# MisterPup/PDE-MultiGrid

Measured on AMD Instinct MI355X. Metric: MLUPS on 3D Poisson 512^3 V-cycle, higher is better.
Workload: dtype f64

## Files before the change

### include/mgx.h

```cpp
#ifndef MGX_H
#define MGX_H

#include <stddef.h>
#include <stdint.h>

#ifdef __cplusplus
extern "C" {
#endif

typedef enum {
    MGX_OK = 0,
    MGX_ERR_INVALID = 1,
    MGX_ERR_SIZE = 2,
    MGX_ERR_HIP = 3,
    MGX_ERR_NOMEM = 4,
    MGX_ERR_RCCL = 5,
    MGX_ERR_NOGPU = 6
} mgx_status;

typedef enum { MGX_RESIDUAL_REF_COMPAT = 0, MGX_RESIDUAL_CORRECT = 1 } mgx_residual_mode;

typedef struct mgx_ctx mgx_ctx;
typedef struct mgx_event mgx_event;

const char* mgx_status_string(int status);
const char* mgx_last_error(void);
void mgx_set_last_error(const char* msg);
const char* mgx_version(void);

int mgx_device_count(int* count);
int mgx_ctx_create(int device, mgx_ctx** out);
int mgx_ctx_destroy(mgx_ctx* ctx);
int mgx_ctx_sync(mgx_ctx* ctx);
int mgx_ctx_check(mgx_ctx* ctx);
int mgx_ctx_clear_abort(mgx_ctx* ctx, int reenable);
int mgx_ctx_generation(const mgx_ctx* ctx, unsigned long long* generation);
int mgx_ctx_prepare(mgx_ctx* ctx);
int mgx_ctx_device(const mgx_ctx* ctx, int* device);
int mgx_ctx_set_param(mgx_ctx* ctx, const char* name, int value);
const char* mgx_ctx_last_relax_kernel(const mgx_ctx* ctx);
const char* mgx_ctx_last_rr_kernel(const mgx_ctx* ctx);
const char* mgx_ctx_last_corr_kernel(const mgx_ctx* ctx);
int mgx_test_set_lds_poison(int on);
int mgx_test_lds_probe(mgx_ctx* ctx, double* fraction);
int mgx_ctx_stream(const mgx_ctx* ctx, void** hip_stream);

int mgx_malloc(mgx_ctx* ctx, size_t bytes, void** dptr);
int mgx_free(mgx_ctx* ctx, void* dptr);
int mgx_memcpy_h2d(mgx_ctx* ctx, void* dst, const void* host_src, size_t bytes);
int mgx_memcpy_d2h(mgx_ctx* ctx, void* host_dst, const void* src, size_t bytes);
int mgx_memcpy_d2d(mgx_ctx* ctx, void* dst, const void* src, size_t bytes);
int mgx_memset_zero(mgx_ctx* ctx, void* dst, size_t bytes);

int mgx_graph_begin(mgx_ctx* ctx);
int mgx_graph_end(mgx_ctx* ctx, void** graph_exec);
int mgx_graph_launch(mgx_ctx* ctx, void* graph_exec);
int mgx_graph_destroy(mgx_ctx* ctx, void* graph_exec);
int mgx_event_create(mgx_ctx* ctx, mgx_event** out);
int mgx_event_destroy(mgx_ctx* ctx, mgx_event* ev);
int mgx_event_record(mgx_ctx* ctx, mgx_event* ev);
int mgx_event_elapsed_ms(mgx_ctx* ctx, mgx_event* start, mgx_event* stop, float* ms);

#define MGX_DECLARE_OPS(SFX, real)                                                                      \
    int mgx3d_relax_##SFX(mgx_ctx* ctx, real* v, const real* f, const int n[3], const real h[3],        \
                          int ncycles);                                                                 \
     \
     \
     \
    int mgx3d_relax_from_zero_##SFX(mgx_ctx* ctx, real* v, const real* f, const int n[3], const real h[3], \
                                    int ncycles, int rim_is_zero);                                      \
    int mgx3d_residual_##SFX(mgx_ctx* ctx, const real* v, const real* f, real* r, const int n[3],       \
                             const real h[3], int mode);                                                \
    int mgx3d_restrict_##SFX(mgx_ctx* ctx, const real* fine, const int fn[3], real* coarse,             \
                             const int cn[3]);                                                          \
    int mgx3d_interpolate_##SFX(mgx_ctx* ctx, real* fine, const int fn[3], const real* coarse,          \
                                const int cn[3]);                                                       \
    int mgx3d_apply_correction_##SFX(mgx_ctx* ctx, real* fine, const int fn[3], const real* err,        \
                                     const int en[3]);                                                  \
    int mgx3d_set_##SFX(mgx_ctx* ctx, real* grid, const int n[3], real value, int modify_boundaries);   \
    int mgx3d_residual_restrict_##SFX(mgx_ctx* ctx, const real* v, const real* f, const int n[3],       \
                                      const real h[3], int mode, real* coarse_f, const int cn[3]);      \
     \
     \
    int mgx3d_residual_restrict_keep_rim_##SFX(mgx_ctx* ctx, const real* v, const real* f,              \
                                               const int n[3], const real h[3], int mode,               \
                                               real* coarse_f, const int cn[3]);                        \
    int mgx3d_interpolate_correct_##SFX(mgx_ctx* ctx, real* v, const int n[3], const real* coarse_v,    \
                                        const int cn[3]);                                               \
    int mgx3d_init_f_##SFX(mgx_ctx* ctx, real* f, const int n[3], double c, const double* host_tx,      \
                           const double* host_ty, const double* host_tz);                               \
    int mgx3d_jacobi_##SFX(mgx_ctx* ctx, real* v, real* tmp, const real* f, const int n[3],             \
                           const real h[3], real omega, int ncycles);                                   \
     \
     \
     \
// ... 286 lines not shown
```

### pde_multigrid_amd/_lib.py

```python
import ctypes as C
import os

_HERE = os.path.dirname(os.path.abspath(__file__))
LIB_PATH = os.environ.get("MGX_LIB_PATH") or os.path.join(_HERE, "lib", "libmgx.so")

MGX_OK, MGX_ERR_INVALID, MGX_ERR_SIZE, MGX_ERR_HIP, MGX_ERR_NOMEM, MGX_ERR_RCCL, MGX_ERR_NOGPU = range(7)
REF_COMPAT, CORRECT = 0, 1
UNIQUE_ID_BYTES = 128


class MgxError(RuntimeError):
    def __init__(self, status, message):
        super().__init__("%s: %s" % (status_string(status), message))
        self.status = status


if not os.path.exists(LIB_PATH):
    raise ImportError(
        "pde_multigrid_amd: %s is missing -- build it with `python -c 'import __graft_entry__ as g; g.build()'` "
        "or `make -C pde_multigrid_amd/csrc`; there is no CPU fallback for the HIP path" % LIB_PATH)

lib = C.CDLL(LIB_PATH, mode=C.RTLD_GLOBAL)
lib.mgx_status_string.restype = C.c_char_p
lib.mgx_last_error.restype = C.c_char_p
lib.mgx_version.restype = C.c_char_p
lib.mgx_ctx_last_relax_kernel.restype = C.c_char_p
lib.mgx_ctx_last_rr_kernel.restype = C.c_char_p
lib.mgx_ctx_last_corr_kernel.restype = C.c_char_p


def status_string(status):
    return lib.mgx_status_string(int(status)).decode()


def check(status):
    if status != MGX_OK:
        raise MgxError(status, lib.mgx_last_error().decode())
    return status
```

### pde_multigrid_amd/csrc/mgx_internal.hpp

```cpp
#pragma once
#include <hip/hip_runtime.h>

#include <cstdarg>
#include <cstdio>
#include <cstring>

#include "mgx.h"

struct mgx_ctx {
    int device = 0;
    hipStream_t compute = nullptr;
    hipStream_t comm = nullptr;
    hipEvent_t ev_compute = nullptr;
    hipEvent_t ev_comm = nullptr;
    int comm_inline = 0;
    int relax_ty = 4;
    int relax_zchunk = 0;
    int relax_xcd = 1;
    int rr_rows = 0;
    int rr_rcp = 1;
    int rr_xcd = 1;
    int relax_rows = 4;
    int relax_wave_planes = 0;
    int relax_small = 1;
    int relax_ablate = 0;
    int rr_stream = 3;
    int relax_lds = -1;
    int rr_cr = 0, rr_tyw = 4;
    int rr_pzchunk = 0;
    int rr_black = 1;
    int rr_black_abl = 0;
    int rr_black_waves = 0;
    int relax_zero_first = 1;
    int relax_zero_sweep = 1;
    int corr_v2 = 1;
    int relax_v2 = 1;
    int corr_fuse = 1;
    int cyc2_tile = 0;
    int cyc2_tail_points = 33 * 33;
    int sweep_fused = 0;
    int sweep_mid = 1;
    int relax_resident = 1;
    int relax_resident_min = 3;
    void* resident_buf = nullptr;
    size_t resident_bytes = 0;
    int sweep_ilv = 0;
    int sweep_lead = 0;
    int sweep_dbg = 0;
    void* sweep_dev = nullptr;
    unsigned* sweep_abort = nullptr;
    unsigned sync_spin_limit = 1u << 21;
    unsigned handoff_fault = 0;
    int handoff_broken = 0;
    unsigned long long generation = 0;
    int gpu_exclusive = 1;
    mutable int resident_occ = -1;
    void* scratch = nullptr;
    size_t scratch_bytes = 0;
    void* rccl_comm = nullptr;
    void* local_group = nullptr;
    int rank = 0, nranks = 1;
    int comm_rehearse = 0;
    void* rehearse_buf = nullptr;
    size_t rehearse_bytes = 0;
    int num_cus = 256;
    int pipe_unroll = 7;
    int corr_low = 0;
    int slab_edges_merged = 1;
    int resident_tile = 0;
    char last_corr_kernel[96] = "";
    char last_rr_kernel[96] = "";
    char last_relax_kernel[96] = "";
};

struct mgx_event {
    hipEvent_t ev = nullptr;
};

namespace mgx {

void set_error(const char* fmt, ...);

inline int fail(int status, const char* fmt, ...) {
    char buf[512];
    va_list ap;
    va_start(ap, fmt);
    vsnprintf(buf, sizeof buf, fmt, ap);
    va_end(ap);
    set_error("%s", buf);
    return status;
}

int workspace(mgx_ctx* ctx, size_t bytes, void** out);
int fill_zero(mgx_ctx* ctx, void* dst, size_t bytes);

inline int ceil_div(long long a, long long b) { return (int)((a + b - 1) / b); }

template <class real>
inline void note_relax_kernel(mgx_ctx* ctx, const char* name, int a, int b, int c, bool fnt = false) {
    snprintf(ctx->last_relax_kernel, sizeof ctx->last_relax_kernel, "%s<%s,%d,%d,%d%s>", name, sizeof(real) == 8 ? "double" : "float",
             a, b, c, fnt ? ",true" : "");
}

inline bool valid_size(int n) { return n >= 3 && ((n - 1) % 2 == 0); }

struct SmallDiv {
    int d;
    float r;
    __host__ __device__ explicit SmallDiv(int d_) : d(d_), r(1.0f / (float)d_) {}
    __device__ __forceinline__ int operator()(int t) const {
        int q = (int)((float)t * r);
        const int rem = t - q * d;
        q += (rem >= d) - (rem < 0);
        return q;
    }
};

}

#define MGX_HIP(expr)                                                                         \
    do {                                                                                      \
        hipError_t e_ = (expr);                                                               \
        if (e_ != hipSuccess)                                                                 \
            return mgx::fail(MGX_ERR_HIP, "%s failed: %s (%s:%d)", #expr, hipGetErrorString(e_), \
                             __FILE__, __LINE__);                                             \
// ... 24 lines not shown
```

### pde_multigrid_amd/csrc/mgx_kernels3d.hip

```cpp
#include <type_traits>

#include "mgx_internal.hpp"
#include "mgx_kernels3d.hpp"
#include "mgx_sync.hpp"

namespace mgx {

template <class real>
__global__ void __launch_bounds__(256) relax3d_colour_kernel(real* __restrict__ v, const real* __restrict__ f, int sx,
                                                             int sy, int sz, real hx2, real hy2, real hz2, int colour) {
    const int y = 1 + blockIdx.y * blockDim.y + threadIdx.y;
    const int z = 1 + blockIdx.z;
    if (y >= sy - 1) return;
    const int p = (colour + y + z) & 1;
    const int x = 2 * (blockIdx.x * blockDim.x + threadIdx.x) + p;
    if (x < 1 || x >= sx - 1) return;
    const size_t sxy = (size_t)sx * sy;
    const size_t i = x + (size_t)y * sx + (size_t)z * sxy;
    const real O = v[i - 1], E = v[i + 1];
    const real N = v[i - sx], S = v[i + sx];
    const real D = v[i - sxy], U = v[i + sxy];
    v[i] = relax3d_point<real>(O, E, N, S, D, U, f[i], hx2, hy2, hz2);
}

// ... 2514 lines not shown
        else if (TYWr == 2) MGX_RR(M, C, 2);       \
        else MGX_RR(M, C, 4);                      \
    } while (0)
    if (mode == MGX_RESIDUAL_REF_COMPAT) {
        if (rcp) { if (CRr == 1) MGX_RR_W(2, 1); else MGX_RR_W(2, 2); }
        else { if (CRr == 1) MGX_RR_W(0, 1); else MGX_RR_W(0, 2); }
    } else {
        if (rcp) { if (CRr == 1) MGX_RR_W(3, 1); else MGX_RR_W(3, 2); }
        else { if (CRr == 1) MGX_RR_W(1, 1); else MGX_RR_W(1, 2); }
    }
#undef MGX_RR_W
#undef MGX_RR
    return MGX_OK;
}

template <class real, class L>
int residual_restrict3d(mgx_ctx* ctx, const real* v, const real* f, const int n[3], const real h[3], int mode,
                        real* coarse_f, const int cn[3], bool rim_is_zero = false) {
    MGX_REQUIRE(ctx && v && f && h && coarse_f, MGX_ERR_INVALID, "residual_restrict3d: NULL argument");
    MGX_USE(ctx);
    int st = check_n3(n, "residual_restrict3d");
    if (st) return st;
    st = check_coarse3(n, cn, "residual_restrict3d");
    if (st) return st;
    MGX_REQUIRE(mode == MGX_RESIDUAL_REF_COMPAT || mode == MGX_RESIDUAL_CORRECT, MGX_ERR_INVALID,
                "residual_restrict3d: bad mode %d", mode);
    const real hx2 = h[0] * h[0], hy2 = h[1] * h[1], hz2 = h[2] * h[2];
    if (L::xsplit && ctx->rr_stream) {
        st = residual_restrict3d_xs_launch<real>(ctx, v, f, n, hx2, hy2, hz2, mode, coarse_f, cn, 0, 0, 0, cn[2], rim_is_zero);
        if (st) return st;
        MGX_LAUNCH_CHECK();
        return MGX_OK;
    }
    constexpr int CTX = 32, CTY = 8;
    const int tiles = ceil_div(cn[0], CTX) * ceil_div(cn[1], CTY);
    int pzchunk = ctx->rr_pzchunk > 0 ? ctx->rr_pzchunk : 8;
    while (pzchunk > 1 && (long long)tiles * ceil_div(cn[2], pzchunk) < 4LL * ctx->num_cus) pzchunk >>= 1;
    dim3 g(ceil_div(cn[0], CTX), ceil_div(cn[1], CTY), ceil_div(cn[2], pzchunk));
    if (mode == MGX_RESIDUAL_REF_COMPAT)
        MGX_LAUNCH((residual_restrict3d_kernel<real, L, 0, CTX, CTY>), g, blk(), 0, ctx->compute, v, f, n[0], n[1],
                           n[2], hx2, hy2, hz2, coarse_f, cn[0], cn[1], cn[2], pzchunk, 0, 0, 0, cn[2]);
    else
        MGX_LAUNCH((residual_restrict3d_kernel<real, L, 1, CTX, CTY>), g, blk(), 0, ctx->compute, v, f, n[0], n[1],
                           n[2], hx2, hy2, hz2, coarse_f, cn[0], cn[1], cn[2], pzchunk, 0, 0, 0, cn[2]);
    MGX_LAUNCH_CHECK();
    return MGX_OK;
}

bool relax_rr3d_xs_takes(const mgx_ctx* ctx, const int n[3], const int cn[3], size_t elem);
template <class real>
bool relax_rr3d_xs_launch(mgx_ctx* ctx, real* v, const real* f, const int n[3], real hx2, real hy2, real hz2, int mode, bool rcp,
                          real* coarse_f, const int cn[3], int fzoff, int czoff, int pzbeg, int pzend);

template <class real>
int relax_rr3d_slab(mgx_ctx* ctx, real* v, const real* f, const int n[3], int fzoff, const real h[3], int mode, real* coarse_f,
                    const int cn[3], int czoff, int pzbeg, int pzend) {
    MGX_REQUIRE(ctx && v && f && h && coarse_f, MGX_ERR_INVALID, "relax_rr_slab: NULL argument");
    MGX_USE(ctx);
    int st = check_n3(n, "relax_rr_slab");
    if (st) return st;
    st = check_coarse3(n, cn, "relax_rr_slab");
    if (st) return st;
    MGX_REQUIRE(mode == MGX_RESIDUAL_REF_COMPAT || mode == MGX_RESIDUAL_CORRECT, MGX_ERR_INVALID, "relax_rr_slab: bad mode %d", mode);
    MGX_REQUIRE(pzbeg >= 1 && pzend <= cn[2] - 1 && pzbeg < pzend && czoff >= 0 && czoff <= pzbeg && fzoff >= 0 && (fzoff & 1) == 0 &&
                    fzoff <= (2 * pzbeg - 3 > 0 ? 2 * pzbeg - 3 : 0),
                MGX_ERR_INVALID, "relax_rr_slab: coarse planes [%d, %d) with offsets %d / %d", pzbeg, pzend, fzoff, czoff);
    MGX_REQUIRE(relax_rr3d_xs_takes(ctx, n, cn, sizeof(real)), MGX_ERR_INVALID, "relax_rr_slab: the level is not taken (ask relax_rr_takes)");
    const real hx2 = h[0] * h[0], hy2 = h[1] * h[1], hz2 = h[2] * h[2];
    const Geo<XSplit, real> gc(cn[0], cn[1]);
    MGX_TRY_RET(fill_zero(ctx, coarse_f + gc.PL * (size_t)(pzbeg - czoff), gc.PL * (size_t)(pzend - pzbeg) * sizeof(real)));
    const bool rcp = ctx->rr_rcp && exact_reciprocal(hx2) && exact_reciprocal(hy2) && exact_reciprocal(hz2);
    MGX_REQUIRE(relax_rr3d_xs_launch<real>(ctx, v, f, n, hx2, hy2, hz2, mode, rcp, coarse_f, cn, fzoff, czoff, pzbeg, pzend), MGX_ERR_INVALID,
                "relax_rr_slab: launch refused");
    MGX_LAUNCH_CHECK();
    return MGX_OK;
}

template <class real>
int smooth_residual_restrict3d_xs(mgx_ctx* ctx, real* v, const real* f, const int n[3], const real h[3], int ncycles, int from_zero,
                                  int v_rim_is_zero, int mode, real* coarse_f, const int cn[3], int coarse_rim_is_zero) {
    MGX_REQUIRE(ctx && v && f && h && coarse_f, MGX_ERR_INVALID, "smooth_residual_restrict3d: NULL argument");
    MGX_USE(ctx);
    int st = check_n3(n, "smooth_residual_restrict3d");
    if (st) return st;
    st = check_coarse3(n, cn, "smooth_residual_restrict3d");
    if (st) return st;
    MGX_REQUIRE(ncycles >= 0, MGX_ERR_INVALID, "smooth_residual_restrict3d: ncycles = %d < 0", ncycles);
    MGX_REQUIRE(mode == MGX_RESIDUAL_REF_COMPAT || mode == MGX_RESIDUAL_CORRECT, MGX_ERR_INVALID,
                "smooth_residual_restrict3d: bad mode %d", mode);
    ctx->last_rr_kernel[0] = 0;
    if (ncycles < 1 || !relax_rr3d_xs_takes(ctx, n, cn, sizeof(real))) {
        st = from_zero ? relax3d_from_zero<real, XSplit>(ctx, v, f, n, h, ncycles, v_rim_is_zero) : relax3d<real, XSplit>(ctx, v, f, n, h, ncycles);
        if (st) return st;
        return residual_restrict3d<real, XSplit>(ctx, v, f, n, h, mode, coarse_f, cn, coarse_rim_is_zero != 0);
    }
    const real hx2 = h[0] * h[0], hy2 = h[1] * h[1], hz2 = h[2] * h[2];
    int s = 0;
    if (from_zero) {
        if (v_rim_is_zero && ctx->relax_zero_first) {
            if (2 * ncycles - 1 >= 2 && relax3d_xs_first_sweep_zero<real>(ctx, v, f, n[0], n[1], n[2], hx2, hy2, hz2)) {
                s = 2;
            } else {
                MGX_LAUNCH((relax3d_zero_colour_kernel<real, XSplit>), dim3(ceil_div((n[0] + 1) / 2, 64), ceil_div(n[1] - 2, 4), n[2] - 2),
                                   blk(), 0, ctx->compute, v, f, n[0], n[1], hx2, hy2, hz2, 0, 1);
                s = 1;
            }
        } else {
            MGX_TRY_RET(fill_zero(ctx, v, Geo<XSplit, real>(n[0], n[1]).PL * (size_t)n[2] * sizeof(real)));
        }
    }
    for (; s < 2 * ncycles - 1; s++) relax3d_xs_pass<real>(ctx, v, f, n[0], n[1], 1, n[2] - 1, hx2, hy2, hz2, s & 1);
    if (!coarse_rim_is_zero) MGX_TRY_RET(fill_zero(ctx, coarse_f, Geo<XSplit, real>(cn[0], cn[1]).PL * (size_t)cn[2] * sizeof(real)));
    const bool rcp = ctx->rr_rcp && exact_reciprocal(hx2) && exact_reciprocal(hy2) && exact_reciprocal(hz2);
    MGX_REQUIRE(relax_rr3d_xs_launch<real>(ctx, v, f, n, hx2, hy2, hz2, mode, rcp, coarse_f, cn, 0, 0, 1, cn[2] - 1), MGX_ERR_INVALID,
                "smooth_residual_restrict3d: the fused launch refused a level it had accepted");
    MGX_LAUNCH_CHECK();
    return MGX_OK;
}

template <class real, class L>
int init_f3d(mgx_ctx* ctx, real* f, const int n[3], double c, const double* tx, const double* ty, const double* tz) {
    MGX_REQUIRE(ctx && f && tx && ty && tz, MGX_ERR_INVALID, "init_f3d: NULL argument");
    MGX_USE(ctx);
    int st = check_n3(n, "init_f3d");
    if (st) return st;
    const size_t cnt = (size_t)n[0] + n[1] + n[2];
    void* ws = nullptr;
    st = workspace(ctx, cnt * sizeof(double), &ws);
    if (st) return st;
    double* d = (double*)ws;
    MGX_HIP(hipMemcpyAsync(d, tx, n[0] * sizeof(double), hipMemcpyHostToDevice, ctx->compute));
    MGX_HIP(hipMemcpyAsync(d + n[0], ty, n[1] * sizeof(double), hipMemcpyHostToDevice, ctx->compute));
    MGX_HIP(hipMemcpyAsync(d + n[0] + n[1], tz, n[2] * sizeof(double), hipMemcpyHostToDevice, ctx->compute));
    MGX_LAUNCH((init_f3d_kernel<real, L>), grd(n[0], n[1], n[2]), blk(), 0, ctx->compute, f, n[0], n[1], n[2], c, d,
                       d + n[0], d + n[0] + n[1]);
    MGX_LAUNCH_CHECK();
    MGX_HIP(hipStreamSynchronize(ctx->compute));
    return MGX_OK;
}

template <class real, class LS, class LD>
int relayout3d(mgx_ctx* ctx, const real* src, real* dst, const int n[3]) {
    MGX_REQUIRE(ctx && src && dst, MGX_ERR_INVALID, "relayout3d: NULL argument");
    MGX_USE(ctx);
    MGX_REQUIRE(src != dst, MGX_ERR_INVALID, "relayout3d: in-place conversion is not supported");
    int st = check_n3(n, "relayout3d");
    if (st) return st;
    MGX_LAUNCH((relayout3d_kernel<real, LS, LD>), grd(n[0], n[1], n[2]), blk(), 0, ctx->compute, src, dst, n[0], n[1]);
    MGX_LAUNCH_CHECK();
    return MGX_OK;
}

template <class real>
int relax3d_colour_slab(mgx_ctx* ctx, real* v, const real* f, int sx, int sy, const real h[3], int colour, int zbeg,
                        int zend, int zoff) {
    MGX_REQUIRE(ctx && v && f && h, MGX_ERR_INVALID, "relax_colour_slab: NULL argument");
    MGX_USE(ctx);
    MGX_REQUIRE(valid_size(sx) && valid_size(sy), MGX_ERR_SIZE, "relax_colour_slab: sizes %d x %d are not odd and >= 3", sx, sy);
    MGX_REQUIRE((colour == 0 || colour == 1) && zbeg >= 1 && zend >= zbeg && zoff >= 0, MGX_ERR_INVALID,
                "relax_colour_slab: bad colour / plane range");
    const real hx2 = h[0] * h[0], hy2 = h[1] * h[1], hz2 = h[2] * h[2];
    relax3d_xs_pass<real>(ctx, v, f, sx, sy, zbeg, zend, hx2, hy2, hz2, (colour + zoff) & 1);
    MGX_LAUNCH_CHECK();
    return MGX_OK;
// ... 570 lines not shown
    int mgx3dxs_relax_rr_takes_##SFX(const mgx_ctx* ctx, const int n[3], const int cn[3]) {                     \
        return ctx && n && cn && mgx::relax_rr3d_xs_takes(ctx, n, cn, sizeof(real));                             \
    }                                                                                                            \
    int mgx3dxs_relax_rr_slab_##SFX(mgx_ctx* ctx, real* v, const real* f, const int n[3], int fzoff,            \
                                    const real h[3], int mode, real* coarse_f, const int cn[3], int czoff,       \
                                    int pzbeg, int pzend) {                                                      \
        return mgx::relax_rr3d_slab<real>(ctx, v, f, n, fzoff, h, mode, coarse_f, cn, czoff, pzbeg, pzend);      \
    }                                                                                                            \
    int mgx3dxs_corr_fused_takes_##SFX(const mgx_ctx* ctx, const int n[3], int nplanes) {                        \
        return ctx && n && mgx::corr_fused_takes(ctx, n[0], n[1], n[2], nplanes);                                \
    }                                                                                                            \
    int mgx3dxs_correct_pset_slab_##SFX(mgx_ctx* ctx, real* v, const int n[3], int fzoff, const real* coarse_v,  \
                                        const int cn[3], int czoff, int zmin, int zmax) {                        \
        return mgx::correct_pset3d_slab<real>(ctx, v, n, fzoff, coarse_v, cn, czoff, zmin, zmax);                \
    }                                                                                                            \
    int mgx3dxs_relax_corr_colour_slab_##SFX(mgx_ctx* ctx, real* v, const real* f, const int n[3], int fzoff,    \
                                             const real h[3], const real* coarse_v, const int cn[3], int czoff,  \
                                             int cplanes, int zbeg, int zend) {                                  \
        return mgx::relax3d_corr_colour_slab<real>(ctx, v, f, n, fzoff, h, coarse_v, cn, czoff, cplanes, zbeg,   \
                                                   zend);                                                        \
    }                                                                                                            \
    int mgx3dxs_interpolate_correct_relax_pp_##SFX(mgx_ctx* ctx, real* v, real* w, const real* f, const int n[3], \
                                                   const real h[3], const real* coarse_v, const int cn[3],       \
                                                   int ncycles, int w_rim_valid) {                               \
        if (!w) return mgx::fail(MGX_ERR_INVALID, "interpolate_correct_relax_pp: w is NULL");                    \
        return mgx::interpolate_correct_relax3d_xs<real>(ctx, v, f, n, h, coarse_v, cn, ncycles, w, w_rim_valid); \
    }                                                                                                            \
    int mgx3dxs_interpolate_correct_colour_##SFX(mgx_ctx* ctx, real* v, const int n[3], const real* coarse_v,    \
                                                 const int cn[3], int colour) {                                  \
        return mgx::interpolate_correct3d_slab<real>(ctx, v, n, 0, coarse_v, cn, 0, 0, cn ? cn[2] - 1 : 0,       \
                                                     colour);                                                    \
    }                                                                                                            \
    int mgx3dxs_pack_##SFX(mgx_ctx* ctx, const real* natural, real* xsplit, const int n[3]) {                    \
        return mgx::relayout3d<real, mgx::Natural, mgx::XSplit>(ctx, natural, xsplit, n);                        \
    }                                                                                                            \
    int mgx3dxs_unpack_##SFX(mgx_ctx* ctx, const real* xsplit, real* natural, const int n[3]) {                  \
        return mgx::relayout3d<real, mgx::XSplit, mgx::Natural>(ctx, xsplit, natural, n);                        \
    }                                                                                                            \
    int mgx_norm2_##SFX(mgx_ctx* ctx, const real* x, size_t count, double* host_sumsq) {                         \
        return mgx::norm2<real>(ctx, x, count, host_sumsq);                                                      \
    }

extern "C" {
MGX_DEFINE_OPS3D(mgx3d_, mgx::Natural, f32, float)
MGX_DEFINE_OPS3D(mgx3d_, mgx::Natural, f64, double)
MGX_DEFINE_OPS3D(mgx3dxs_, mgx::XSplit, f32, float)
MGX_DEFINE_OPS3D(mgx3dxs_, mgx::XSplit, f64, double)
MGX_DEFINE_MISC3D(f32, float)
MGX_DEFINE_MISC3D(f64, double)

const char* mgx_ctx_last_relax_kernel(const mgx_ctx* ctx) { return ctx ? ctx->last_relax_kernel : ""; }
const char* mgx_ctx_last_rr_kernel(const mgx_ctx* ctx) { return ctx ? ctx->last_rr_kernel : ""; }
const char* mgx_ctx_last_corr_kernel(const mgx_ctx* ctx) { return ctx ? ctx->last_corr_kernel : ""; }

int mgx_ctx_set_param(mgx_ctx* ctx, const char* name, int value) {
    MGX_REQUIRE(ctx && name, MGX_ERR_INVALID, "set_param: NULL argument");
    MGX_USE(ctx);
    ctx->generation++;
    if (!strcmp(name, "relax3d.ty")) {
        MGX_REQUIRE(value == 1 || value == 2 || value == 4 || value == 8, MGX_ERR_INVALID, "relax3d.ty (waves per block) must be 1, 2, 4 or 8");
        ctx->relax_ty = value;
    } else if (!strcmp(name, "relax3d.small")) {
        ctx->relax_small = value ? 1 : 0;
    } else if (!strcmp(name, "relax3d.ablate")) {
#ifdef MGX_DIAGNOSTICS
        ctx->relax_ablate = value;
#else
        return mgx::fail(MGX_ERR_INVALID, "set_param: 'relax3d.ablate' exists only in diagnostic builds (make diag)");
#endif
    } else if (!strcmp(name, "relax3d.wave_planes")) {
        ctx->relax_wave_planes = value;
    } else if (!strcmp(name, "relax3d.rows")) {
        MGX_REQUIRE(value == 1 || value == 2 || value == 4 || value == 8, MGX_ERR_INVALID, "relax3d.rows must be 1, 2, 4 or 8");
        ctx->relax_rows = value;
    } else if (!strcmp(name, "residual_restrict3d.rows")) {
        MGX_REQUIRE(value == 0 || value == 2 || value == 4, MGX_ERR_INVALID, "residual_restrict3d.rows (fine rows per wave of the pipelined kernel) must be 0 (by level size), 2 or 4");
        ctx->rr_rows = value;
    } else if (!strcmp(name, "residual_restrict3d.rcp")) {
        MGX_REQUIRE(value == 0 || value == 1, MGX_ERR_INVALID, "residual_restrict3d.rcp must be 0 or 1");
        ctx->rr_rcp = value;
    } else if (!strcmp(name, "residual_restrict3d.xcd")) {
        MGX_REQUIRE(value >= 0 && value <= 2, MGX_ERR_INVALID, "residual_restrict3d.xcd must be 0, 1 or 2");
        ctx->rr_xcd = value;
    } else if (!strcmp(name, "relax3d.xcd")) {
        MGX_REQUIRE(value >= 0 && value <= 2, MGX_ERR_INVALID, "relax3d.xcd must be 0, 1 or 2");
        ctx->relax_xcd = value;
    } else if (!strcmp(name, "relax3d.lds")) {
        bool ok = value == -1 || value == 0 || value == 3282 || (value >= 1000 && value < 2000 && mgx::relax3d_lds_shape_known(value - 1000));
#ifdef MGX_DIAGNOSTICS
        ok = ok || (value > 0 && value < 1000 && mgx::relax3d_lds_shape_known(value)) || (value >= 3000 && mgx::relax3d_lds_shape_known(value - 3000));
#endif
        MGX_REQUIRE(ok, MGX_ERR_INVALID, "relax3d.lds = %d is not a kernel shape of this build", value);
        ctx->relax_lds = value;
    } else if (!strcmp(name, "residual_restrict3d.cr")) {
        MGX_REQUIRE(value >= 0 && value <= 2, MGX_ERR_INVALID, "residual_restrict3d.cr must be 0 (by level size), 1 or 2");
        ctx->rr_cr = value;
    } else if (!strcmp(name, "residual_restrict3d.tyw")) {
        MGX_REQUIRE(value == 2 || value == 4 || value == 8, MGX_ERR_INVALID, "residual_restrict3d.tyw (waves per block) must be 2, 4 or 8");
        ctx->rr_tyw = value;
    } else if (!strcmp(name, "residual_restrict3d.stream")) {
        MGX_REQUIRE(value >= 0 && value <= 3, MGX_ERR_INVALID, "residual_restrict3d.stream must be 0 ... 3");
        ctx->rr_stream = value;
    } else if (!strcmp(name, "residual_restrict3d.pzchunk")) {
        MGX_REQUIRE(value >= 0, MGX_ERR_INVALID, "residual_restrict3d.pzchunk must be >= 0 (0 = automatic)");
        ctx->rr_pzchunk = value;
    } else if (!strcmp(name, "relax3d.zero_first")) {
// ... 19 lines not shown
    } else if (!strcmp(name, "relax3d.resident")) {
        MGX_REQUIRE(value >= 0 && value <= 2, MGX_ERR_INVALID, "set_param: relax3d.resident = %d not in {0, 1, 2}", value);
        ctx->relax_resident = value;
    } else if (!strcmp(name, "sync.spin_limit")) {
        MGX_REQUIRE(value >= 1, MGX_ERR_INVALID, "set_param: sync.spin_limit = %d < 1", value);
        ctx->sync_spin_limit = (unsigned)value;
    } else if (!strcmp(name, "test.handoff_fault")) {
        MGX_REQUIRE(value >= 0 && value < (1 << 20), MGX_ERR_INVALID, "set_param: test.handoff_fault = %d out of range", value);
        ctx->handoff_fault = (unsigned)value;
    } else if (!strcmp(name, "gpu.exclusive")) {
        MGX_REQUIRE(value == 0 || value == 1, MGX_ERR_INVALID, "set_param: gpu.exclusive = %d not in {0, 1}", value);
        ctx->gpu_exclusive = value;
    } else if (!strcmp(name, "relax3d.corr_low")) {
        MGX_REQUIRE(value == 0 || value == 1, MGX_ERR_INVALID, "set_param: relax3d.corr_low = %d not in {0, 1}", value);
        ctx->corr_low = value;
    } else if (!strcmp(name, "slab.edges_merged")) {
        MGX_REQUIRE(value == 0 || value == 1, MGX_ERR_INVALID, "set_param: slab.edges_merged = %d not in {0, 1}", value);
        ctx->slab_edges_merged = value;
    } else if (!strcmp(name, "relax3d.resident_tile")) {
        MGX_REQUIRE(value == 0 || value == 8, MGX_ERR_INVALID, "set_param: relax3d.resident_tile = %d not in {0, 8}", value);
        ctx->resident_tile = value;
    } else if (!strcmp(name, "relax3d.resident_min")) {
        MGX_REQUIRE(value >= 1, MGX_ERR_INVALID, "set_param: relax3d.resident_min = %d < 1", value);
        ctx->relax_resident_min = value;
    } else if (!strcmp(name, "rr3d.black")) {
        MGX_REQUIRE(value >= 0 && value <= 2, MGX_ERR_INVALID, "set_param: rr3d.black = %d not in {0, 1, 2}", value);
        ctx->rr_black = value;
    } else if (!strcmp(name, "rr3d.black_waves")) {
        MGX_REQUIRE(value == 0 || value == 8 || value == 12 || value == 16, MGX_ERR_INVALID, "set_param: rr3d.black_waves = %d not in {0, 8, 12, 16}", value);
        ctx->rr_black_waves = value;
    } else if (!strcmp(name, "rr3d.black_abl")) {
#ifdef MGX_DIAGNOSTICS
        ctx->rr_black_abl = value;
#else
        return mgx::fail(MGX_ERR_INVALID, "set_param: 'rr3d.black_abl' exists only in diagnostic builds (make diag)");
#endif
    } else if (!strcmp(name, "relax3d.fused_ilv")) {
        ctx->sweep_ilv = value ? 1 : 0;
    } else if (!strcmp(name, "relax3d.fused_mid")) {
        MGX_REQUIRE(value >= 0 && value <= 2, MGX_ERR_INVALID, "set_param: relax3d.fused_mid = %d not in {0, 1, 2}", value);
        ctx->sweep_mid = value;
    } else if (!strcmp(name, "relax3d.fused_dbg")) {
#ifdef MGX_DIAGNOSTICS
        ctx->sweep_dbg = value;
#else
        return mgx::fail(MGX_ERR_INVALID, "set_param: 'relax3d.fused_dbg' exists only in diagnostic builds (make diag)");
#endif
    } else if (!strcmp(name, "relax3d.fused_lead")) {
        MGX_REQUIRE(value == 0 || (value >= 5 && value <= 7), MGX_ERR_INVALID, "relax3d.fused_lead (planes the red stage runs ahead) must be 0 (default), 5, 6 or 7");
        ctx->sweep_lead = value;
    } else if (!strcmp(name, "relax3d.unroll")) {
        MGX_REQUIRE(value >= 0 && value <= 31, MGX_ERR_INVALID, "set_param: relax3d.unroll = %d not in [0, 31]", value);
        ctx->pipe_unroll = value;
    } else if (!strcmp(name, "relax3d.zchunk")) {
        MGX_REQUIRE(value >= 0, MGX_ERR_INVALID, "relax3d.zchunk must be >= 0 (0 = automatic)");
        ctx->relax_zchunk = value;
    } else {
        return mgx::fail(MGX_ERR_INVALID, "set_param: unknown parameter '%s'", name);
    }
    return MGX_OK;
}
}
```

### pde_multigrid_amd/multigrid.py

```python
import ctypes as C

import numpy as np

from ._lib import REF_COMPAT, check, lib


def _ct(dtype):
    dtype = np.dtype(dtype)
    if dtype == np.float32:
        return "f32", C.c_float
    if dtype == np.float64:
        return "f64", C.c_double
    raise TypeError("dtype must be float32 or float64, got %s" % dtype)


def _ip(a):
    return (C.c_int * len(a))(*[int(x) for x in a])


def _rp(a, ct):
    return (ct * len(a))(*[float(x) for x in a])


def _shape(n):
# ... 7 lines not shown
    return c


def num_grids(min_size):
    return lib.mg_num_grids(int(min_size))


def coarse_size(n):
    return tuple(lib.mg_coarse_size(int(k)) for k in n)


def grid_spacing(n, rng, dtype):
    t = np.dtype(dtype).type
    return [t(t(rng[2 * d + 1]) - t(rng[2 * d])) / t(int(n[d]) - 1) for d in range(len(n))]


class Context:

    def __init__(self, device=0):
        self._h = C.c_void_p()
        check(lib.mgx_ctx_create(int(device), C.byref(self._h)))
        self.device = int(device)

    def close(self):
        if self._h:
            lib.mgx_ctx_destroy(self._h)
            self._h = C.c_void_p()

    def __del__(self):
        try:
            self.close()
        except Exception:
            pass

    def sync(self):
        check(lib.mgx_ctx_sync(self._h))

    def malloc(self, nbytes):
        p = C.c_void_p()
        check(lib.mgx_malloc(self._h, C.c_size_t(int(nbytes)), C.byref(p)))
        return p

    def free(self, p):
        check(lib.mgx_free(self._h, p))

    def last_relax_kernel(self):
        return lib.mgx_ctx_last_relax_kernel(self._h).decode()

    def last_rr_kernel(self):
        return lib.mgx_ctx_last_rr_kernel(self._h).decode()

    def last_corr_kernel(self):
        return lib.mgx_ctx_last_corr_kernel(self._h).decode()

    def set_param(self, name, value):
        check(lib.mgx_ctx_set_param(self._h, name.encode(), C.c_int(int(value))))

    def generation(self):
        g = C.c_ulonglong()
        check(lib.mgx_ctx_generation(self._h, C.byref(g)))
        return int(g.value)

    def clear_abort(self, reenable=False):
        check(lib.mgx_ctx_clear_abort(self._h, C.c_int(1 if reenable else 0)))

    def to_device(self, arr):
        arr = np.ascontiguousarray(arr)
        p = self.malloc(arr.nbytes)
        check(lib.mgx_memcpy_h2d(self._h, p, arr.ctypes.data_as(C.c_void_p), C.c_size_t(arr.nbytes)))
        return p

    def to_host(self, p, shape, dtype):
        out = np.empty(shape, dtype)
        check(lib.mgx_memcpy_d2h(self._h, out.ctypes.data_as(C.c_void_p), p, C.c_size_t(out.nbytes)))
        return out

    def event(self):
        e = C.c_void_p()
        check(lib.mgx_event_create(self._h, C.byref(e)))
        return e

    def record(self, e):
        check(lib.mgx_event_record(self._h, e))

    def elapsed_ms(self, e0, e1):
        ms = C.c_float()
        check(lib.mgx_event_elapsed_ms(self._h, e0, e1, C.byref(ms)))
        return float(ms.value)

    @staticmethod
    def unique_id():
        buf = (C.c_ubyte * 128)()
        check(lib.mgx_comm_unique_id(buf))
        return bytes(buf)

    def comm_init(self, unique_id, rank, nranks):
        buf = (C.c_ubyte * 128).from_buffer_copy(unique_id)
        check(lib.mgx_comm_init(self._h, buf, int(rank), int(nranks)))

    def comm_init_rehearsal(self, unique_id, virtual_rank, virtual_nranks):
        buf = (C.c_ubyte * 128).from_buffer_copy(unique_id)
        check(lib.mgx_comm_init_rehearsal(self._h, buf, int(virtual_rank), int(virtual_nranks)))

    def comm_info(self):
        n, v = C.c_int(0), C.c_int(0)
        check(lib.mgx_comm_info(self._h, C.byref(n), C.byref(v)))
# ... 156 lines not shown

    def residual(self, ctx, v, f, n, rng, mode=REF_COMPAT, dtype=None):
        dtype = dtype or v.dtype
        fn, ct = self._fn("residual", dtype)
        h = _rp(grid_spacing(n, rng, dtype), ct)
        r = np.zeros(_shape(n), dtype)
        return self._run(ctx, [v, f, r], lambda a, b, c: fn(ctx._h, a, b, c, _ip(n), h, C.c_int(mode)), 2, _shape(n), dtype)

    def residual_restrict(self, ctx, v, f, n, rng, mode=REF_COMPAT, dtype=None):
        dtype = dtype or v.dtype
        fn, ct = self._fn("residual_restrict", dtype)
        h = _rp(grid_spacing(n, rng, dtype), ct)
        cn = coarse_size(n)
        coarse = np.zeros(_shape(cn), dtype)
        return self._run(ctx, [v, f, coarse], lambda a, b, c: fn(ctx._h, a, b, _ip(n), h, C.c_int(mode), c, _ip(cn)), 2,
                         _shape(cn), dtype)

    def interpolate_correct(self, ctx, v, n, coarse, dtype=None):
        dtype = dtype or v.dtype
        fn, _ = self._fn("interpolate_correct", dtype)
        cn = coarse_size(n)
        return self._run(ctx, [v, coarse], lambda a, c: fn(ctx._h, a, _ip(n), c, _ip(cn)), 0, _shape(n), dtype)

    def interpolate_correct_colour(self, ctx, v, n, coarse, colour, dtype=None):
        dtype = dtype or v.dtype
        fn, _ = self._fn("interpolate_correct_colour", dtype)
        cn = coarse_size(n)
        return self._run(ctx, [v, coarse], lambda a, c: fn(ctx._h, a, _ip(n), c, _ip(cn), C.c_int(colour)), 0, _shape(n), dtype)

    def relax_from_zero(self, ctx, v, f, n, rng, ncycles, rim_is_zero, dtype=None):
        dtype = dtype or v.dtype
        fn, ct = self._fn("relax_from_zero", dtype)
        h = _rp(grid_spacing(n, rng, dtype), ct)
        return self._run(ctx, [v, f], lambda a, b: fn(ctx._h, a, b, _ip(n), h, C.c_int(ncycles), C.c_int(int(rim_is_zero))), 0, _shape(n),
                         dtype)

    def smooth_residual_restrict(self, ctx, v, f, n, rng, ncycles, from_zero=False, v_rim_is_zero=False, mode=REF_COMPAT, dtype=None):
        dtype = dtype or v.dtype
        fn, ct = self._fn("smooth_residual_restrict", dtype)
        h = _rp(grid_spacing(n, rng, dtype), ct)
        cn = coarse_size(n)
        pv, pf = ctx.to_device(xs_pack(np.ascontiguousarray(v, dtype))), ctx.to_device(xs_pack(np.ascontiguousarray(f, dtype)))
        pc = ctx.to_device(xs_pack(np.full(_shape(cn), np.nan, dtype)))
        try:
            check(fn(ctx._h, pv, pf, _ip(n), h, C.c_int(ncycles), C.c_int(int(from_zero)), C.c_int(int(v_rim_is_zero)), C.c_int(mode), pc,
                     _ip(cn), C.c_int(0)))
            isz = np.dtype(dtype).itemsize
            out_v = xs_unpack(ctx.to_host(pv, tuple(_shape(n)[:-1]) + (xs_geometry(n[0], isz)[1],), dtype), n[0])
            out_c = xs_unpack(ctx.to_host(pc, tuple(_shape(cn)[:-1]) + (xs_geometry(cn[0], isz)[1],), dtype), cn[0])
            return out_v, out_c
        finally:
            for q in (pv, pf, pc):
                ctx.free(q)

    def interpolate_correct_relax(self, ctx, v, f, n, rng, coarse, ncycles, dtype=None):
        dtype = dtype or v.dtype
        fn, ct = self._fn("interpolate_correct_relax", dtype)
        h = _rp(grid_spacing(n, rng, dtype), ct)
        cn = coarse_size(n)
        return self._run(ctx, [v, f, coarse], lambda a, b, c: fn(ctx._h, a, b, _ip(n), h, c, _ip(cn), C.c_int(ncycles)), 0, _shape(n),
                         dtype)

    def jacobi(self, ctx, v, f, n, rng, omega, ncycles, dtype=None):
        dtype = dtype or v.dtype
        fn, ct = self._fn("jacobi", dtype)
        h = _rp(grid_spacing(n, rng, dtype), ct)
        return self._run(ctx, [v, np.zeros_like(v), f], lambda a, t, b: fn(ctx._h, a, t, b, _ip(n), h, ct(omega), C.c_int(ncycles)),
                         0, _shape(n), dtype)

    def norm2(self, ctx, x):
        s, _ = _ct(x.dtype)
        out = C.c_double()
        p = ctx.to_device(x)
        try:
            check(getattr(lib, "mgx_norm2_" + s)(ctx._h, p, C.c_size_t(x.size), C.byref(out)))
        finally:
            ctx.free(p)
        return float(out.value)


    def _krylov_work(self, ctx, n, dtype):
        s, _ = _ct(dtype)
        fn = getattr(lib, "mgx3dxs_krylov_work_elems_" + s)
        fn.restype = C.c_size_t
        return ctx.to_device(np.zeros(max(int(fn(_ip(n))), 1), np.float64))

    def _krylov(self, ctx, n, arrays, scalars, call, dtype, nsum):
        assert self.xsplit, "the Krylov kernels exist for the x-split layout only"
        work = self._krylov_work(ctx, n, dtype)
        dev = [ctx.to_device(np.array(scalars + [0.0] * nsum, np.float64))]
        ptrs = [ctx.to_device(a) if a is not None else None for a in arrays]
        try:
            sp = [C.c_void_p(dev[0].value + 8 * i) for i in range(len(scalars) + nsum)]
            check(call(work, *sp, *ptrs))
            sums = ctx.to_host(dev[0], (len(scalars) + nsum,), np.float64)[len(scalars):]
            return [ctx.to_host(p, a.shape, dtype) if p is not None else None for p, a in zip(ptrs, arrays)], sums
        finally:
            for p in ptrs + dev + [work]:
                if p is not None:
                    ctx.free(p)

    def laplace_dot(self, ctx, p, n, rng, q=None, packed=False, dtype=None):
        dtype = dtype or p.dtype
        fn, ct = self._fn("laplace_dot", dtype)
        h = _rp(grid_spacing(n, rng, dtype), ct)
        pp = p if packed else xs_pack(np.ascontiguousarray(p, dtype))
# ... 631 lines not shown
```

Baseline: 193,700.

## Add fused three-sweep temporally blocked red-black relax kernel for f64

Adds a kernel that performs three consecutive red-black half-sweeps in one pass over z, keeping intermediate planes in registers and LDS with y-halo overlap. It replaces the last three separate relax passes before residual-restrict for large f64 grids, so each of those passes no longer streams the full grid from memory on its own. In exchange it recomputes halo rows, adds barriers and register pressure, and runs the kernel in place over v.

Result: faster. 215,500, median of 6 (+11.3%).

```diff
diff --git a/include/mgx.h b/include/mgx.h
--- a/include/mgx.h
+++ b/include/mgx.h
@@ -41,6 +41,9 @@
 const char* mgx_ctx_last_relax_kernel(const mgx_ctx* ctx);
 const char* mgx_ctx_last_rr_kernel(const mgx_ctx* ctx);
 const char* mgx_ctx_last_corr_kernel(const mgx_ctx* ctx);
+const char* mgx_ctx_last_block3_kernel(const mgx_ctx* ctx);
+int mgx3dxs_relax_block3_f64(mgx_ctx* ctx, const double* vin, double* vout, const double* f, const int n[3], const double h[3],
+                             int first_colour, int store_both);
 int mgx_test_set_lds_poison(int on);
 int mgx_test_lds_probe(mgx_ctx* ctx, double* fraction);
 int mgx_ctx_stream(const mgx_ctx* ctx, void** hip_stream);
diff --git a/pde_multigrid_amd/_lib.py b/pde_multigrid_amd/_lib.py
--- a/pde_multigrid_amd/_lib.py
+++ b/pde_multigrid_amd/_lib.py
@@ -27,6 +27,7 @@
 lib.mgx_ctx_last_relax_kernel.restype = C.c_char_p
 lib.mgx_ctx_last_rr_kernel.restype = C.c_char_p
 lib.mgx_ctx_last_corr_kernel.restype = C.c_char_p
+lib.mgx_ctx_last_block3_kernel.restype = C.c_char_p
 
 
 def status_string(status):
diff --git a/pde_multigrid_amd/csrc/mgx_block3d.hip b/pde_multigrid_amd/csrc/mgx_block3d.hip
--- /dev/null
+++ b/pde_multigrid_amd/csrc/mgx_block3d.hip
@@ -0,0 +1,234 @@
+#include <type_traits>
+
+#include "mgx_internal.hpp"
+#include "mgx_kernels3d.hpp"
+
+namespace mgx {
+
+template <class real, int COL, bool STORE_BOTH, int TW>
+__global__ void __launch_bounds__(64 * TW, 4)
+    relax3d_xs_block3_kernel(const real* vin, real* vout, const real* __restrict__ f, int sx, int sy, int sz, real hx2, real hy2,
+                             real hz2, int zrun, int gx, int gy, int xcd_mode) {
+    constexpr int ROWS = 2 * TW, OUTR = ROWS - 6;
+    static_assert(OUTR % 2 == 0, "the colour parity of a wave's rows must not depend on the tile");
+    __shared__ real sY[2][TW][2][64];
+    __shared__ real sX[2][TW][2][64];
+    __shared__ real sZ[2][TW][2][64];
+    const Geo<XSplit, real> g(sx, sy);
+    const int lane = threadIdx.x;
+    const int w = __builtin_amdgcn_readfirstlane(threadIdx.y);
+    int bx, by, bz;
+    tile_of_block(xcd_mode, gx, gy, bx, by, bz);
+    const int z0 = 1 + bz * zrun, z1 = min(z0 + zrun, sz - 1);
+    if (z0 >= z1) return;
+    const int PL = (int)g.PL;
+
+    const int Hn = (sx + 1) >> 1;
+    const int pn = bx * 60 + lane - 2, p = min(max(pn, 0), Hn - 1);
+    const unsigned off0 = (unsigned)p * (unsigned)sizeof(real), off1 = (unsigned)(g.H + (p <= Hn - 2 ? p : 0)) * (unsigned)sizeof(real);
+    const bool xin0 = pn >= 1 && 2 * pn <= sx - 2, xin1 = pn >= 0 && 2 * pn + 1 <= sx - 2;
+    auto off = [&](int h) { return h ? off1 : off0; };
+    auto xin = [&](int h) { return h ? xin1 : xin0; };
+    const bool xface0 = pn <= 0 || pn >= Hn - 1;
+    const bool wxface = bx * 60 - 2 <= 0 || bx * 60 + 61 >= Hn - 1;
+    const bool outlane = lane >= 2 && lane <= 61;
+    int roff[2];
+    bool yin[2], outrow[2];
+#pragma unroll
+    for (int o = 0; o < 2; o++) {
+        const int y = by * OUTR - 3 + 2 * w + o;
+        roff[o] = min(max(y, 0), sy - 1) * g.P;
+        yin[o] = y >= 1 && y <= sy - 2;
+        outrow[o] = 2 * w + o >= 3 && 2 * w + o < ROWS - 3;
+    }
+    const int wU = w > 0 ? w - 1 : 0, wD = w < TW - 1 ? w + 1 : TW - 1;
+    auto zc = [&](int z) { return min(max(z, 0), sz - 1); };
+    auto plane = [&](const real* a, int z) { return plane_rsrc<real>(a + (ptrdiff_t)zc(z) * (ptrdiff_t)g.PL, PL, 1); };
+
+    real a_m[2], a_c[2], a_p[2], a_n[2], fx_c[2], fx_1[2], fx_2[2], fx_n[2], xv_n[2], fy_c[2], fy_n[2];
+    real b_c[2], b_m[2], b_mm[2], d_c[2], d_m[2], d_mm[2], x3[2];
+#pragma unroll
+    for (int o = 0; o < 2; o++)
+        a_m[o] = a_c[o] = a_p[o] = a_n[o] = fx_c[o] = fx_1[o] = fx_2[o] = fx_n[o] = xv_n[o] = fy_c[o] = fy_n[o] = b_c[o] =
+            b_m[o] = b_mm[o] = d_c[o] = d_m[o] = d_mm[o] = x3[o] = 0;
+
+    const int t0 = z0 - 2, tlast = z1 + 1;
+    {
+        const auto qm = plane(vin, t0 - 1), q0 = plane(vin, t0), qp = plane(vin, t0 + 1);
+        const bool zf = t0 <= 0 || t0 >= sz - 1;
+        const auto qf = plane(f, t0);
+#pragma unroll
+        for (int o = 0; o < 2; o++) {
+            const int hx = (COL + 1 + o + t0) & 1;
+            a_m[o] = buf_load<real>(qm, off(hx), roff[o]);
+            a_c[o] = buf_load<real>(q0, off(hx ^ 1), roff[o]);
+            a_p[o] = buf_load<real>(qp, off(hx), roff[o]);
+            fx_c[o] = buf_load<real>(zf || !yin[o] ? q0 : qf, off(hx), roff[o]);
+            if (wxface) xv_n[o] = buf_load<real>(q0, off(0), roff[o]);
+        }
+        __builtin_amdgcn_s_waitcnt(0x0F70);
+#pragma unroll
+        for (int o = 0; o < 2; o++)
+            if (wxface && ((COL + 1 + o + t0) & 1) == 0 && xface0) fx_c[o] = xv_n[o];
+        const int b = (t0 - 1) & 1;
+        sY[b][w][0][lane] = a_c[0];
+        sY[b][w][1][lane] = a_c[1];
+        asm volatile("s_waitcnt lgkmcnt(0)\n\ts_barrier" ::: "memory");
+    }
+
+    auto relax = [&](auto hc, int o, const real (&c)[2], real nb, real sb, real D, real U, real fv) __attribute__((always_inline)) {
+        constexpr int h = decltype(hc)::value;
+        real O, E;
+        if (h == 0) {
+            O = wave_from_prev_lane<real>(c[o]);
+            E = c[o];
+        } else {
+            O = c[o];
+            E = wave_from_next_lane<real>(c[o]);
+        }
+        const real N = o == 0 ? nb : c[0], S = o == 1 ? sb : c[1];
+        return relax3d_point<real>(O, E, N, S, D, U, fv, hx2, hy2, hz2);
+    };
+
+    auto iteration = [&](auto parity, int t) __attribute__((always_inline)) {
+        constexpr int PAR = decltype(parity)::value;
+        constexpr int PB = PAR ^ 1;
+        const auto ro3 = plane(vout, t - 3), ro2 = plane(vout, t - 2);
+        const auto rY = plane(vin, t + 2), rXv = plane(vin, t + 1), rFx = plane(f, t + 1), rFy = plane(f, t);
+        const bool zf = t + 1 <= 0 || t + 1 >= sz - 1;
+        __builtin_amdgcn_s_setprio(3);
+#pragma unroll
+        for (int o = 0; o < 2; o++) {
+            const int hx = (COL + 1 + o + PAR) & 1;
+            const bool sto = outlane && yin[o] && outrow[o];
+            if (t - 3 >= z0 && t - 3 < z1 && sto && xin(hx ^ 1)) buf_store_nt<real>(x3[o], ro3, off(hx ^ 1), roff[o]);
+            if (STORE_BOTH && t - 2 >= z0 && t - 2 < z1 && sto && xin(hx ^ 1)) buf_store_nt<real>(d_m[o], ro2, off(hx ^ 1), roff[o]);
+            a_n[o] = buf_load<real>(rY, off(hx ^ 1), roff[o]);
+            fx_n[o] = buf_load<real>(zf || !yin[o] ? rXv : rFx, off(hx ^ 1), roff[o]);
+            if ((hx ^ 1) == 0 && wxface) xv_n[o] = buf_load<real>(rXv, off(0), roff[o]);
+            fy_n[o] = buf_load<real>(rFy, off(hx ^ 1), roff[o]);
+        }
+        __builtin_amdgcn_s_setprio(0);
+        const bool zin1 = t >= 1 && t <= sz - 2, zin2 = t - 1 >= 1 && t - 1 <= sz - 2;
+        {
+            const real nb = sY[PB][wU][1][lane], sb = sY[PB][wD][0][lane];
+#pragma unroll
+            for (int o = 0; o < 2; o++) {
+                const real v1 = (((COL + 1 + PAR) & 1) ^ o) == 0
+                                    ? relax(std::integral_constant<int, 0>{}, o, a_c, nb, sb, a_m[o], a_p[o], fx_c[o])
+                                    : relax(std::integral_constant<int, 1>{}, o, a_c, nb, sb, a_m[o], a_p[o], fx_c[o]);
+                const int hx = (COL + 1 + o + PAR) & 1;
+                b_c[o] = zin1 && yin[o] && xin(hx) ? v1 : fx_c[o];
+            }
+        }
+        {
+            const real nb = sX[PB][wU][1][lane], sb = sX[PB][wD][0][lane];
+#pragma unroll
+            for (int o = 0; o < 2; o++) {
+                const real v2 = (((COL + 1 + PAR) & 1) ^ o) == 0
+                                    ? relax(std::integral_constant<int, 0>{}, o, b_m, nb, sb, b_mm[o], b_c[o], fy_c[o])
+                                    : relax(std::integral_constant<int, 1>{}, o, b_m, nb, sb, b_mm[o], b_c[o], fy_c[o]);
+                const int hx = (COL + 1 + o + PAR) & 1;
+                d_c[o] = zin2 && yin[o] && xin(hx) ? v2 : a_m[o];
+            }
+        }
+        {
+            const real nb = sZ[PB][wU][1][lane], sb = sZ[PB][wD][0][lane];
+#pragma unroll
+            for (int o = 0; o < 2; o++) {
+                x3[o] = (((COL + 1 + PAR) & 1) ^ o) == 0
+                            ? relax(std::integral_constant<int, 0>{}, o, d_m, nb, sb, d_mm[o], d_c[o], fx_2[o])
+                            : relax(std::integral_constant<int, 1>{}, o, d_m, nb, sb, d_mm[o], d_c[o], fx_2[o]);
+            }
+        }
+#pragma unroll
+        for (int o = 0; o < 2; o++) {
+            sY[PAR][w][o][lane] = a_p[o];
+            sX[PAR][w][o][lane] = b_c[o];
+            sZ[PAR][w][o][lane] = d_c[o];
+        }
+        asm volatile("s_waitcnt lgkmcnt(0)\n\ts_barrier" ::: "memory");
+        __builtin_amdgcn_s_waitcnt(0x0F70);
+#pragma unroll
+        for (int o = 0; o < 2; o++) {
+            a_m[o] = a_c[o]; a_c[o] = a_p[o]; a_p[o] = a_n[o];
+            fx_2[o] = fx_1[o]; fx_1[o] = fx_c[o];
+            fx_c[o] = ((COL + 1 + o + PAR) & 1) == 1 && wxface && xface0 ? xv_n[o] : fx_n[o];
+            fy_c[o] = fy_n[o];
+            b_mm[o] = b_m[o]; b_m[o] = b_c[o];
+            d_mm[o] = d_m[o]; d_m[o] = d_c[o];
+        }
+    };
+
+    int t = t0;
+    if (t & 1) iteration(std::integral_constant<int, 1>{}, t++);
+    for (;; t += 2) {
+        iteration(std::integral_constant<int, 0>{}, t);
+        if (t == tlast) break;
+        iteration(std::integral_constant<int, 1>{}, t + 1);
+        if (t + 1 == tlast) break;
+    }
+    {
+        const auto ro3 = plane(vout, tlast - 2);
+#pragma unroll
+        for (int o = 0; o < 2; o++) {
+            const int hx = (COL + 1 + o + tlast) & 1;
+            if (outlane && yin[o] && outrow[o] && xin(hx)) buf_store_nt<real>(x3[o], ro3, off(hx), roff[o]);
+        }
+    }
+}
+
+bool relax_block3_takes(const mgx_ctx* ctx, const int n[3], size_t elem, int part) {
+    if (!(ctx->block3 & part) || elem != 8) return false;
+    if ((unsigned long long)Geo<XSplit, double>(n[0], n[1]).PL * 8ull >= (1ull << 31)) return false;
+    return n[0] >= 385 && n[1] >= 129 && n[2] >= 65;
+}
+
+template <class real>
+void relax3d_xs_block3_launch(mgx_ctx* ctx, const real* vin, real* vout, const real* f, const int n[3], real hx2, real hy2, real hz2,
+                              int first_colour, bool store_both) {
+    constexpr int TW = 16;
+    const int gx = ceil_div((n[0] - 1) / 2, 60), gy = ceil_div(n[1] - 2, 2 * TW - 6);
+    const int tiles = gx * gy, planes = n[2] - 2;
+    int nchunks = 1;
+    double best = 0;
+    for (int c = 1; c <= 64 && (c == 1 || planes / c >= 16); c++) {
+        const long long wgs = (long long)tiles * c, cap = ctx->num_cus;
+        const double eff = (double)wgs / (double)(((wgs + cap - 1) / cap) * cap) * (double)planes / (double)(planes + 4 * c);
+        if (eff > best + 1e-9) { best = eff; nchunks = c; }
+        if (eff >= 0.9) break;
+    }
+    const int zrun = ceil_div(planes, nchunks);
+    const dim3 grid(tiles * ceil_div(planes, zrun), 1, 1), blk(64, TW, 1);
+#define MGX_B3(C, S)                                                                                                          \
+    MGX_LAUNCH((relax3d_xs_block3_kernel<real, C, S, TW>), grid, blk, 0, ctx->compute, vin, vout, f, n[0], n[1], n[2], hx2, hy2, \
+               hz2, zrun, gx, gy, 1)
+    if (first_colour == 0) {
+        if (store_both) MGX_B3(0, true); else MGX_B3(0, false);
+    } else {
+        if (store_both) MGX_B3(1, true); else MGX_B3(1, false);
+    }
+#undef MGX_B3
+    snprintf(ctx->last_block3_kernel, sizeof ctx->last_block3_kernel, "relax3d_xs_block3_kernel<%s,%d,%s,%d>",
+             sizeof(real) == 8 ? "double" : "float", first_colour, store_both ? "true" : "false", TW);
+}
+template void relax3d_xs_block3_launch<double>(mgx_ctx*, const double*, double*, const double*, const int[3], double, double, double, int,
+                                               bool);
+
+}
+
+extern "C" int mgx3dxs_relax_block3_f64(mgx_ctx* ctx, const double* vin, double* vout, const double* f, const int n[3], const double h[3],
+                                        int first_colour, int store_both) {
+    MGX_REQUIRE(ctx && vin && vout && f && n && h, MGX_ERR_INVALID, "relax_block3: NULL argument");
+    MGX_USE(ctx);
+    MGX_REQUIRE(mgx::valid_size(n[0]) && mgx::valid_size(n[1]) && mgx::valid_size(n[2]), MGX_ERR_SIZE,
+                "relax_block3: sizes %d x %d x %d are not odd and >= 3", n[0], n[1], n[2]);
+    MGX_REQUIRE(first_colour == 0 || first_colour == 1, MGX_ERR_INVALID, "relax_block3: first_colour = %d not in {0, 1}", first_colour);
+    const unsigned long long plane_bytes = (unsigned long long)mgx::Geo<mgx::XSplit, double>(n[0], n[1]).PL * 8ull;
+    MGX_REQUIRE(plane_bytes < (1ull << 31), MGX_ERR_SIZE,
+                "relax_block3: a plane of %d x %d is too large", n[0], n[1]);
+    MGX_REQUIRE(!store_both || vin != vout, MGX_ERR_INVALID, "relax_block3: store_both needs vout != vin");
+    mgx::relax3d_xs_block3_launch<double>(ctx, vin, vout, f, n, h[0] * h[0], h[1] * h[1], h[2] * h[2], first_colour, store_both != 0);
+    MGX_LAUNCH_CHECK();
+    return MGX_OK;
+}
diff --git a/pde_multigrid_amd/csrc/mgx_internal.hpp b/pde_multigrid_amd/csrc/mgx_internal.hpp
--- a/pde_multigrid_amd/csrc/mgx_internal.hpp
+++ b/pde_multigrid_amd/csrc/mgx_internal.hpp
@@ -71,6 +71,8 @@
     char last_corr_kernel[96] = "";
     char last_rr_kernel[96] = "";
     char last_relax_kernel[96] = "";
+    int block3 = 1;
+    char last_block3_kernel[96] = "";
 };
 
 struct mgx_event {
diff --git a/pde_multigrid_amd/csrc/mgx_kernels3d.hip b/pde_multigrid_amd/csrc/mgx_kernels3d.hip
--- a/pde_multigrid_amd/csrc/mgx_kernels3d.hip
+++ b/pde_multigrid_amd/csrc/mgx_kernels3d.hip
@@ -2590,6 +2590,13 @@
 bool relax_rr3d_xs_launch(mgx_ctx* ctx, real* v, const real* f, const int n[3], real hx2, real hy2, real hz2, int mode, bool rcp,
                           real* coarse_f, const int cn[3], int fzoff, int czoff, int pzbeg, int pzend);
 
+bool relax_block3_takes(const mgx_ctx* ctx, const int n[3], size_t elem, int part);
+template <class real>
+void relax3d_xs_block3_launch(mgx_ctx* ctx, const real* vin, real* vout, const real* f, const int n[3], real hx2, real hy2, real hz2,
+                              int first_colour, bool store_both);
+template <>
+void relax3d_xs_block3_launch<float>(mgx_ctx*, const float*, float*, const float*, const int[3], float, float, float, int, bool) {}
+
 template <class real>
 int relax_rr3d_slab(mgx_ctx* ctx, real* v, const real* f, const int n[3], int fzoff, const real h[3], int mode, real* coarse_f,
                     const int cn[3], int czoff, int pzbeg, int pzend) {
@@ -2627,6 +2634,7 @@
     MGX_REQUIRE(mode == MGX_RESIDUAL_REF_COMPAT || mode == MGX_RESIDUAL_CORRECT, MGX_ERR_INVALID,
                 "smooth_residual_restrict3d: bad mode %d", mode);
     ctx->last_rr_kernel[0] = 0;
+    ctx->last_block3_kernel[0] = 0;
     if (ncycles < 1 || !relax_rr3d_xs_takes(ctx, n, cn, sizeof(real))) {
         st = from_zero ? relax3d_from_zero<real, XSplit>(ctx, v, f, n, h, ncycles, v_rim_is_zero) : relax3d<real, XSplit>(ctx, v, f, n, h, ncycles);
         if (st) return st;
@@ -2647,7 +2655,9 @@
             MGX_TRY_RET(fill_zero(ctx, v, Geo<XSplit, real>(n[0], n[1]).PL * (size_t)n[2] * sizeof(real)));
         }
     }
-    for (; s < 2 * ncycles - 1; s++) relax3d_xs_pass<real>(ctx, v, f, n[0], n[1], 1, n[2] - 1, hx2, hy2, hz2, s & 1);
+    const bool b3 = !from_zero && 2 * ncycles - 1 - s >= 3 && relax_block3_takes(ctx, n, sizeof(real), 1);
+    for (; s < 2 * ncycles - 1 - (b3 ? 3 : 0); s++) relax3d_xs_pass<real>(ctx, v, f, n[0], n[1], 1, n[2] - 1, hx2, hy2, hz2, s & 1);
+    if (b3) relax3d_xs_block3_launch<real>(ctx, v, v, f, n, hx2, hy2, hz2, 0, false);
     if (!coarse_rim_is_zero) MGX_TRY_RET(fill_zero(ctx, coarse_f, Geo<XSplit, real>(cn[0], cn[1]).PL * (size_t)cn[2] * sizeof(real)));
     const bool rcp = ctx->rr_rcp && exact_reciprocal(hx2) && exact_reciprocal(hy2) && exact_reciprocal(hz2);
     MGX_REQUIRE(relax_rr3d_xs_launch<real>(ctx, v, f, n, hx2, hy2, hz2, mode, rcp, coarse_f, cn, 0, 0, 1, cn[2] - 1), MGX_ERR_INVALID,
@@ -3324,6 +3334,7 @@
 const char* mgx_ctx_last_relax_kernel(const mgx_ctx* ctx) { return ctx ? ctx->last_relax_kernel : ""; }
 const char* mgx_ctx_last_rr_kernel(const mgx_ctx* ctx) { return ctx ? ctx->last_rr_kernel : ""; }
 const char* mgx_ctx_last_corr_kernel(const mgx_ctx* ctx) { return ctx ? ctx->last_corr_kernel : ""; }
+const char* mgx_ctx_last_block3_kernel(const mgx_ctx* ctx) { return ctx ? ctx->last_block3_kernel : ""; }
 
 int mgx_ctx_set_param(mgx_ctx* ctx, const char* name, int value) {
     MGX_REQUIRE(ctx && name, MGX_ERR_INVALID, "set_param: NULL argument");
@@ -3449,6 +3460,9 @@
     } else if (!strcmp(name, "relax3d.unroll")) {
         MGX_REQUIRE(value >= 0 && value <= 31, MGX_ERR_INVALID, "set_param: relax3d.unroll = %d not in [0, 31]", value);
         ctx->pipe_unroll = value;
+    } else if (!strcmp(name, "relax3d.block3")) {
+        MGX_REQUIRE(value == 0 || value == 1, MGX_ERR_INVALID, "set_param: relax3d.block3 = %d not in {0, 1}", value);
+        ctx->block3 = value;
     } else if (!strcmp(name, "relax3d.zchunk")) {
         MGX_REQUIRE(value >= 0, MGX_ERR_INVALID, "relax3d.zchunk must be >= 0 (0 = automatic)");
         ctx->relax_zchunk = value;
diff --git a/pde_multigrid_amd/multigrid.py b/pde_multigrid_amd/multigrid.py
--- a/pde_multigrid_amd/multigrid.py
+++ b/pde_multigrid_amd/multigrid.py
@@ -83,6 +83,9 @@
 
     def last_corr_kernel(self):
         return lib.mgx_ctx_last_corr_kernel(self._h).decode()
+
+    def last_block3_kernel(self):
+        return lib.mgx_ctx_last_block3_kernel(self._h).decode()
 
     def set_param(self, name, value):
         check(lib.mgx_ctx_set_param(self._h, name.encode(), C.c_int(int(value))))
@@ -345,6 +348,15 @@
         finally:
             for q in (pv, pf, pc):
                 ctx.free(q)
+
+    def relax_block3(self, ctx, vin, f, n, rng, first_colour=0, store_both=False, vout=None):
+        h = _rp(grid_spacing(n, rng, np.float64), C.c_double)
+        arrs = [vin, f] if vout is None else [vin, f, vout]
+        if vout is None:
+            call = lambda a, b: lib.mgx3dxs_relax_block3_f64(ctx._h, a, a, b, _ip(n), h, C.c_int(first_colour), C.c_int(int(store_both)))
+            return self._run(ctx, arrs, call, 0, _shape(n), np.float64)
+        call = lambda a, b, c: lib.mgx3dxs_relax_block3_f64(ctx._h, a, c, b, _ip(n), h, C.c_int(first_colour), C.c_int(int(store_both)))
+        return self._run(ctx, arrs, call, 2, _shape(n), np.float64)
 
     def interpolate_correct_relax(self, ctx, v, f, n, rng, coarse, ncycles, dtype=None):
         dtype = dtype or v.dtype
```
